# DhayaaAnbajagane/Baryonification

Hardware: AMD Instinct MI355X
Metric: halos/sec for BaryonifyShell NSIDE=1024 (1000000-halo synthetic catalog) (higher is better)
Workload: dtype f64 throughout in the parity-grade mode: f64 ring-row geometry, f64 pair math with 1e-11 elementary functions (fp32 seeds + one Newton step), f64 LDS accumulation, pix_offsets stored as two f32 arrays (hi + lo), f64 regrid geometry, f64 map

## Files before the change

### baryonification_amd/csrc/bfgx_regrid2.hpp

```cpp
#pragma once
#include "bfgx_kernels.hpp"
#include "bfgx_scatter2.hpp"

namespace bfgx {

template <typename real>
struct alignas(16) RegRowC {
    real z, sth, dphi, inv_dphi;
    real c0, s0;
    real inv_dth_up, inv_dth_dn;
};
template <>
struct alignas(16) RegRowC<double> { double inv_dth_up, inv_dth_dn; };
template <typename real> struct RowGeom { real z, sth, dphi, inv_dphi, c0, s0, inv_dth_up, inv_dth_dn; };
__device__ inline RowGeom<float> row_geom(const RegRow *, const RegRowC<float> *rowc, int t)
{
    const RegRowC<float> c = rowc[t];
    return RowGeom<float>{c.z, c.sth, c.dphi, c.inv_dphi, c.c0, c.s0, c.inv_dth_up, c.inv_dth_dn};
}
__device__ inline RowGeom<double> row_geom(const RegRow *rows, const RegRowC<double> *rowc, int t)
{
    const RegRow &r = rows[t];
    const RegRowC<double> c = rowc[t];
    return RowGeom<double>{r.z, r.sth, r.dphi, r.inv_dphi, r.c0, r.s0, c.inv_dth_up, c.inv_dth_dn};
}
__device__ inline float row_inv_dphi(const RegRow *, const RegRowC<float> *rowc, int t) { return rowc[t].inv_dphi; }
__device__ inline double row_inv_dphi(const RegRow *rows, const RegRowC<double> *, int t) { return rows[t].inv_dphi; }
__host__ __device__ inline size_t regrowc_bytes(size_t real_size) { return real_size == 4 ? sizeof(RegRowC<float>) : sizeof(RegRowC<double>); }

__device__ inline void regrid_targets_generic(const Hpx &h, const RegRow *rows, int LR, int rth0, int ti, int x,
                                                    double o0, double o1, double o2, int tr[4], int tk[4], double w[4])
{
    const int nl4 = (int)(4 * h.nside);
    const RegRow &rw = rows[ti];
    const double z = rw.z, sth = rw.sth;
    const double phi = ((double)(rw.ks + x) + (rw.shf ? 0.5 : 0.0)) * rw.dphi;
    double s, c;
    sincos_bounded(phi, s, c);
    const double nx = sth * c + o0, ny = sth * s + o1, nz = z + o2;
    const double xr = nx * c + ny * s, yr = ny * c - nx * s;
    const double inv = fast_rsq(nx * nx + ny * ny + nz * nz);
    const double zc = nz * inv;
    const double tq = yr * fast_rcp(xr);
    const double sn = fast_sqrt(xr * xr + yr * yr) * inv;
    const double q = sn * z - zc * sth;
    double theta, ph;
    if (xr > 0.0 && fabs(tq) <= 0.1 && fabs(q) <= 0.05) {
        ph = phi + atan_small(tq);
        theta = rw.theta + asin_small(q);
    } else {
        theta = atan2_generic(sn, zc);
        ph = atan2_generic(ny, nx);
    }
    if (ph < 0) ph += kTwoPi;
    if (ph >= kTwoPi) ph -= kTwoPi;
    int t1 = ti;
    while (t1 > 0 && theta < rows[t1].theta) --t1;
    while (t1 < LR + 1 && theta >= rows[t1 + 1].theta) ++t1;
    const bool in_window = (theta >= rows[t1].theta) && (t1 < LR + 1) && (theta < rows[t1 + 1].theta);
    const int ir1 = in_window ? rth0 + t1 : (int)ring_above(h, zc);
    const int ir2 = ir1 + 1;
    double theta1 = 0.0, theta2 = 0.0;
    for (int q4 = 0; q4 < 4; ++q4) { tr[q4] = 0; tk[q4] = 0; w[q4] = 0.0; }
#pragma unroll
    for (int half = 0; half < 2; ++half) {
        const int ir = half ? ir2 : ir1;
        if (half ? (ir < nl4) : (ir > 0)) {
            const int t2 = ir - rth0;
            int n2; double shd, invd, th;
            if (t2 >= 0 && t2 < LR + 2) {
                const RegRow &r2 = rows[t2];
                n2 = r2.nr; shd = r2.shf ? 0.5 : 0.0; invd = r2.inv_dphi; th = r2.theta;
            } else {
                n2 = ring_len(h, ir);
                const bool sh2 = (ir < h.nside) || (ir >= 3 * h.nside) || (((ir - (int)h.nside) & 1) == 0);
                shd = sh2 ? 0.5 : 0.0; invd = (double)n2 * kInvTwoPi; th = ring_theta_nolibm(h, ir);
            }
            const double tmp = ph * invd - shd;
            int j1 = (int)floor(tmp);
            const double w1 = tmp - (double)j1;
            int j2 = j1 + 1;
            if (j1 < 0) j1 += n2;
            if (j2 >= n2) j2 -= n2;
            tr[2 * half] = ir; tr[2 * half + 1] = ir;
            tk[2 * half] = j1; tk[2 * half + 1] = j2;
            w[2 * half] = 1.0 - w1; w[2 * half + 1] = w1;
            if (half) theta2 = th; else theta1 = th;
        }
    }
    if (ir1 == 0) {
        const double wtheta = theta / theta2;
        w[2] *= wtheta; w[3] *= wtheta;
        const double fac = (1.0 - wtheta) * 0.25;
        w[0] = fac; w[1] = fac; w[2] += fac; w[3] += fac;
        tr[0] = 1; tr[1] = 1; tk[0] = (tk[2] + 2) & 3; tk[1] = (tk[3] + 2) & 3;
    } else if (ir2 == nl4) {
        const double wtheta = (theta - theta1) / (kPi - theta1);
        w[0] *= (1.0 - wtheta); w[1] *= (1.0 - wtheta);
        const double fac = wtheta * 0.25;
        w[0] += fac; w[1] += fac; w[2] = fac; w[3] = fac;
        tr[2] = nl4 - 1; tr[3] = nl4 - 1; tk[2] = (tk[0] + 2) & 3; tk[3] = (tk[1] + 2) & 3;
    } else {
        const double wtheta = (theta - theta1) * fast_rcp(theta2 - theta1);
        w[0] *= (1.0 - wtheta); w[1] *= (1.0 - wtheta);
        w[2] *= wtheta; w[3] *= wtheta;
    }
}

__device__ inline float abs_(float v) { return __builtin_fabsf(v); }
__device__ inline double abs_(double v) { return __builtin_fabs(v); }
template <typename real> struct RMath;
template <> struct RMath<float> {
    static __device__ inline float rcp(float x) { const float y = __builtin_amdgcn_rcpf(x); return y * __builtin_fmaf(-x, y, 2.0f); }
    static __device__ inline float inv_norm(float e) { return fma_(e, fma_(e, fma_(e, fma_(e, 0.2734375f, -0.3125f), 0.375f), -0.5f), 1.0f); }
    static __device__ inline float sqrt1pm1(float t2) { return t2 * fma_(t2, fma_(t2, 0.0625f, -0.125f), 0.5f); }
    static __device__ inline float asin_(float q) { const float q2 = q * q; return q * fma_(q2, fma_(q2, fma_(q2, (float)(15.0 / 336.0), 0.075f), (float)(1.0 / 6.0)), 1.0f); }
    static __device__ inline float atan_(float t) { const float t2 = t * t; return t * fma_(t2, fma_(t2, fma_(t2, fma_(t2, (float)(1.0 / 9.0), (float)(-1.0 / 7.0)), 0.2f), (float)(-1.0 / 3.0)), 1.0f); }
};
template <> struct RMath<double> {
    static __device__ inline double rcp(double x) { return fast_rcp(x); }
    static __device__ inline double inv_norm(double e) { return fast_rsq(1.0 + e); }
    static __device__ inline double sqrt1pm1(double t2) { const double h = 1.0 + t2; return t2 * fast_rcp(1.0 + h * fast_rsq(h)); }
    static __device__ inline double asin_(double q) { return asin_small(q); }
    static __device__ inline double atan_(double t) { return atan_small(t); }
};

struct RMathE {
    static __device__ inline double rcp(double x) { const double y = (double)__builtin_amdgcn_rcpf((float)x); return __builtin_fma(y, __builtin_fma(-x, y, 1.0), y); }
    static __device__ inline double inv_norm(double e)
    {
        const double x = 1.0 + e, y = (double)__builtin_amdgcn_rsqf((float)x);
        const double h = 0.5 * y, r = __builtin_fma(-x * y, h, 0.5);
        return __builtin_fma(y, r, y);
    }
    static __device__ inline double sqrt1pm1(double t2) { return t2 * __builtin_fma(t2, __builtin_fma(t2, __builtin_fma(t2, __builtin_fma(t2, 7.0 / 256.0, -5.0 / 128.0), 0.0625), -0.125), 0.5); }
    static __device__ inline double asin_(double q) { const double q2 = q * q; return q * __builtin_fma(q2, __builtin_fma(q2, __builtin_fma(q2, 15.0 / 336.0, 0.075), 1.0 / 6.0), 1.0); }
    static __device__ inline double atan_(double t)
    {
        const double t2 = t * t;
        return t * __builtin_fma(t2, __builtin_fma(t2, __builtin_fma(t2, __builtin_fma(t2, __builtin_fma(t2, -1.0 / 11.0, 1.0 / 9.0), -1.0 / 7.0), 0.2), -1.0 / 3.0), 1.0);
    }
};

constexpr int kReachMax = 16;
constexpr int kReachColsMax = 256;

__host__ __device__ inline double regrid_cap(int64_t nside)
{
    const double c = 9.9 / (double)nside;
    return c < 0.02 ? c : 0.02;
}
__host__ __device__ inline int regrid_reach_rings(int64_t nside, double m)
{
    const double r = m * 1.5 * (double)nside;
    const int R = (r < (double)kReachMax ? (int)r : kReachMax) + 1;
    return R > kReachMax ? kReachMax : R;
}
__host__ __device__ inline double regrid_cap_for_rings(int64_t nside, int R)
{
    const double c = 0.999 * (double)R / (1.5 * (double)nside), cap = regrid_cap(nside);
    return (R >= kReachMax || c > cap) ? cap : c;
}

struct alignas(16) RowScan {
    int32_t start, nr, ks, span;
    float need2, cf2, lim2;
    int32_t klr;
};

struct FarList {
    unsigned long long *count;
    int64_t *pix;
    double *val;
    int64_t cap;
    int32_t *overflow;
};

struct ReachArgs {
    const int32_t *apron;
    double cap;
    double theta_first, theta_last;
};

constexpr int kWalkQ = 128;
constexpr int kWalkFar = (256 / kWave) * kWalkQ;
__host__ __device__ inline size_t regrid3_lds_bytes(int BR, int W, size_t real_size, bool walk = false, size_t acc_size = 0)
{
    if (acc_size == 0) acc_size = real_size;
    const size_t base = (size_t)BR * W * sizeof(double) + (size_t)(BR + 2 * kReachMax + 2) * (sizeof(RegRow) + regrowc_bytes(real_size)) + 16;
    if (!walk) return base;
    return base + (size_t)(BR + 2 * kReachMax + 2) * sizeof(RowScan) + (size_t)(256 / kWave) * kWalkQ * (sizeof(double) + sizeof(int32_t) + 3 * acc_size)
           + (size_t)(kWalkFar + 4) * sizeof(int32_t);
}

template <typename ACC>
__global__ void __launch_bounds__(256)
tile_reach_kernel(Hpx h, Tiling T, const ACC *__restrict__ offsets, float *__restrict__ tile_omax)
{
    __shared__ float red[256 / kWave];
    const int tile = blockIdx.x;
    const int band = T.tile_band[tile];
    const int nphi = T.band_nphi[band];
    const int tj = tile - T.band_tile0[band];
    const int nl4 = (int)(4 * h.nside);
    const int i0 = 1 + band * T.BR, i1 = min(i0 + T.BR, nl4);
    const int lane = threadIdx.x & (kWave - 1), wid = threadIdx.x / kWave;
    float m2 = 0.0f;
    for (int ring = i0 + wid; ring < i1; ring += 256 / kWave) {
        int64_t st, nr64; bool shf;
        ring_info_small(h, ring, st, nr64, shf);
        const int nr = (int)nr64, ks = tile_ks(tj, nr, nphi), ke = tile_ks(tj + 1, nr, nphi);
        const ACC *o = offsets + 3 * (st + ks);
        for (int x = lane; x < ke - ks; x += kWave) {
            const float a = (float)o[3 * x], b = (float)o[3 * x + 1], c = (float)o[3 * x + 2];
            m2 = fmaxf(m2, fma_(a, a, fma_(b, b, c * c)));
        }
    }
#pragma unroll
    for (int sft = kWave >> 1; sft > 0; sft >>= 1) m2 = fmaxf(m2, __shfl_down(m2, sft, kWave));
    if (lane == 0) red[wid] = m2;
    __syncthreads();
    if (threadIdx.x == 0) {
        for (int w = 1; w < 256 / kWave; ++w) m2 = fmaxf(m2, red[w]);
        tile_omax[tile] = m2;
    }
}

__global__ void __launch_bounds__(256)
tile_apron_kernel(Hpx h, Tiling T, const float *__restrict__ tile_omax, int rings, double cap, int tile0, int ntiles,
                  int32_t *__restrict__ apron, int32_t *__restrict__ todo, int32_t *__restrict__ lean = nullptr)
{
    const int i = blockIdx.x * 256 + threadIdx.x;
    bool is_lean = false;
    if (i < ntiles) {
    const int tile = tile0 + i;
    const int band = T.tile_band[tile];
    const int nphi = T.band_nphi[band];
    const int tj = tile - T.band_tile0[band];
    const int nl4 = (int)(4 * h.nside);
    float m = (float)cap;
    int R = rings;
    if (tile_omax != nullptr) {
        m = 0.0f;
        const int nb = (kReachMax + T.BR - 1) / T.BR;
        for (int db = -nb; db <= nb; ++db) {
            const int b2 = band + db;
            if (b2 < 0 || b2 >= T.nbands) continue;
            const int n2 = T.band_nphi[b2], t20 = T.band_tile0[b2];
            int lo = (int)(((int64_t)tj * n2) / nphi) - 1, hi = (int)(((int64_t)(tj + 1) * n2 + nphi - 1) / nphi) + 1;
            if (T.W < 32 || hi - lo >= n2) { lo = 0; hi = n2; }
            for (int t2 = lo; t2 < hi; ++t2) {
                const int u = t2 < 0 ? t2 + n2 : (t2 >= n2 ? t2 - n2 : t2);
                m = fmaxf(m, tile_omax[t20 + u]);
            }
        }
        const bool still = !(m > 0.0f);
        m = fminf(__builtin_sqrtf(m) * 1.001f, (float)cap);
        R = still ? 0 : regrid_reach_rings(h.nside, (double)m);
    }
    const int i0 = 1 + band * T.BR, i1 = min(i0 + T.BR, nl4);
    const int rlo = max(i0 - R, 1), rhi = min(i1 + R, nl4) - 1, ns = (int)h.nside;
    int nmin = 0x7fffffff, nmax = 0;
    float mc = 0.0f;
    const int probe[4] = {rlo, rhi, ns, 3 * ns};
#pragma unroll
    for (int q = 0; q < 4; ++q) {
        const int ring = probe[q];
        if (ring < rlo || ring > rhi) continue;
        double z, sth;
        ring_z_sth(h, ring, z, sth);
        const int nr = ring_len(h, ring);
        nmin = min(nmin, nr); nmax = max(nmax, nr);
        const float limf = fminf(m, (float)(0.09 * sth)), den = (float)sth - limf;
        if (den > 0.0f) mc = fmaxf(mc, limf / den * 1.02f * (float)nr * (float)kInvTwoPi);
    }
    const float kk = mc + (float)nmax / (float)nmin + 2.5f;
    apron[2 * tile] = R;
    apron[2 * tile + 1] = (nphi == 1) ? 0 : (kk < (float)kReachColsMax ? (int)kk + 1 : kReachColsMax);
    if (todo != nullptr && R > 1) todo[1 + atomicAdd(todo, 1)] = tile;
    is_lean = R <= 1;
    }
    if (lean != nullptr) {
        const unsigned long long m = __ballot(is_lean);
        if (m) {
            const int lane = threadIdx.x & (kWave - 1), leader = __ffsll((long long)m) - 1;
            int base = 0;
            if (lane == leader) base = atomicAdd(lean, __popcll(m));
            base = __shfl(base, leader, kWave);
            const int pos = base + __popcll(m & ((1ull << lane) - 1ull));
            if (is_lean && pos < ntiles) lean[1 + pos] = tile0 + i;
        }
    }
}

template <typename ACC>
__global__ void __launch_bounds__(256)
max_offset_kernel(int64_t n, const ACC *__restrict__ offsets, unsigned *__restrict__ out)
{
    float m2 = 0.0f;
    for (int64_t i = (int64_t)blockIdx.x * 256 + threadIdx.x; i < n; i += (int64_t)gridDim.x * 256) {
        const float a = (float)offsets[3 * i], b = (float)offsets[3 * i + 1], c = (float)offsets[3 * i + 2];
        m2 = fmaxf(m2, fma_(a, a, fma_(b, b, c * c)));
    }
#pragma unroll
    for (int sft = kWave >> 1; sft > 0; sft >>= 1) m2 = fmaxf(m2, __shfl_down(m2, sft, kWave));
    __shared__ float wm[256 / kWave];
    if ((threadIdx.x & (kWave - 1)) == 0) wm[threadIdx.x / kWave] = m2;
    __syncthreads();
    if (threadIdx.x == 0) {
        float m = 0.0f;
        for (int w = 0; w < 256 / kWave; ++w) m = fmaxf(m, wm[w]);
        if (m > 0.0f) atomicMax(out, __float_as_uint(m));
    }
}

__global__ void __launch_bounds__(1024)
max_bits_kernel(int n, const unsigned *__restrict__ v, unsigned *__restrict__ out)
{
    unsigned m = 0u;
    for (int i = threadIdx.x; i < n; i += 1024) m = max(m, v[i]);
#pragma unroll
    for (int sft = kWave >> 1; sft > 0; sft >>= 1) m = max(m, (unsigned)__shfl_down((int)m, sft, kWave));
    if ((threadIdx.x & (kWave - 1)) == 0 && m) atomicMax(out, m);
}

template <typename real, bool WALK, bool ECON = false>
__device__ inline bool regrid_gather_targets(const RegRow *rows, const RegRowC<real> *rowc, int NT, int ti, int x,
                                             real o0, real o1, real o2, int tt[4], int tk[4], real w[4])
{
    using RM = typename std::conditional<ECON, RMathE, RMath<real>>::type;
    using PMx = typename std::conditional<ECON, PMathE, PMath<real>>::type;
    const RowGeom<real> rc = row_geom(rows, rowc, ti);
    const RegRow &rw = rows[ti];
    real c, s;
    const real alpha = (real)x * rc.dphi;
    if (abs_(alpha) <= (real)0.45) {
        real sa, oma;
        PMx::sin_omc(alpha, sa, oma);
        c = rc.c0 - (rc.c0 * oma + rc.s0 * sa);
        s = rc.s0 - (rc.s0 * oma - rc.c0 * sa);
    } else {
        double s64, c64;
        sincos_bounded(((double)(rw.ks + x) + (rw.shf ? 0.5 : 0.0)) * rw.dphi, s64, c64);
        c = (real)c64; s = (real)s64;
    }
    const real a = o0 * c + o1 * s, b = o1 * c - o0 * s;
    const real xr = rc.sth + a;
    const real t = b * RM::rcp(xr);
    const real t2 = t * t;
    const real e = (real)2 * (rc.sth * a + rc.z * o2) + (a * a + b * b + o2 * o2);
    const real invn = RM::inv_norm(e);
    const real q = (fma_(a, rc.z, -(o2 * rc.sth)) + xr * rc.z * RM::sqrt1pm1(t2)) * invn;
    const real dth = RM::asin_(q);
    const real dph = RM::atan_(t);
    const bool down = dth >= (real)0;
    const real wq = down ? dth * rc.inv_dth_dn : -dth * rc.inv_dth_up;
    int t1 = ti;
    real wtheta;
    const bool near = wq < (real)1 && (down ? rc.inv_dth_dn : rc.inv_dth_up) > (real)0;
    if (!WALK || near) {
        wtheta = down ? wq : (real)1 - wq;
    } else {
        const double d = (double)dth, th0 = rw.theta;
        const int stp = (int)(wq < (real)(2 * kReachMax) ? wq : (real)(2 * kReachMax));
        t1 = down ? ti + stp : ti - 1 - stp;
        t1 = t1 < 0 ? 0 : (t1 > NT - 2 ? NT - 2 : t1);
        while (t1 + 2 < NT && d >= rows[t1 + 1].theta - th0) ++t1;
        while (t1 > 0 && d < rows[t1].theta - th0) --t1;
        const double lo = rows[t1].theta - th0, hi = rows[t1 + 1].theta - th0;
        if (!(d >= lo && d < hi) || rows[t1].nr == 0 || rows[t1 + 1].nr == 0) return false;
        wtheta = (real)((d - lo) * fast_rcp(hi - lo));
    }
    const int nro = rw.nr;
    int kown = rw.ks + x;
    if (kown < 0) kown += nro;
    if (kown >= nro) kown -= nro;
    auto other_ring = [&](int tr, int &j, real &wj) {
        const RegRow &rn = rows[tr];
        const double B = ((double)kown + (rw.shf ? 0.5 : 0.0)) * ((double)rn.nr * rw.dphi * kInvTwoPi) - (rn.shf ? 0.5 : 0.0);
        const double Bf = floor(B);
        const real wall = (real)(B - Bf) + dph * row_inv_dphi(rows, rowc, tr), f = __builtin_floor(wall);
        wj = wall - f; j = (int)Bf + (int)f;
    };
    const bool nr_ = !WALK || near;
    const bool x_upper = !nr_ || down;
    const int tx = nr_ ? ti : t1, ty = nr_ ? (down ? ti + 1 : ti - 1) : t1 + 1;
    int jx, jy; real wx, wy;
    if (nr_) {
        const real wall = dph * rc.inv_dphi, f = __builtin_floor(wall);
        wx = wall - f; jx = kown + (int)f;
    } else {
        other_ring(tx, jx, wx);
    }
    other_ring(ty, jy, wy);
    const int nrx = rows[tx].nr, nry = rows[ty].nr;
    int jx2 = jx + 1, jy2 = jy + 1;
    jx = jx < 0 ? jx + nrx : (jx >= nrx ? jx - nrx : jx);
    jx2 = jx2 < 0 ? jx2 + nrx : (jx2 >= nrx ? jx2 - nrx : jx2);
    jy = jy < 0 ? jy + nry : (jy >= nry ? jy - nry : jy);
    jy2 = jy2 < 0 ? jy2 + nry : (jy2 >= nry ? jy2 - nry : jy2);
    const real wtx = x_upper ? (real)1 - wtheta : wtheta, wty = (real)1 - wtx;
    tt[0] = tx; tt[1] = tx; tk[0] = jx; tk[1] = jx2;
    w[0] = ((real)1 - wx) * wtx; w[1] = wx * wtx;
    tt[2] = ty; tt[3] = ty; tk[2] = jy; tk[3] = jy2;
    w[2] = ((real)1 - wy) * wty; w[3] = wy * wty;
    return true;
}

__device__ inline double regrid_far_pixel(
    const Hpx &h, const RegRow *rows, int LR, int rth0, int ti, int x, double o0, double o1, double o2,
                                                double val, FarList far)
{
    int tr[4], tk[4];
    double w[4], tot = 0.0;
    regrid_targets_generic(h, rows, LR, rth0, ti, x, o0, o1, o2, tr, tk, w);
    const unsigned long long act = __ballot(1);
    const int rank = (int)__builtin_amdgcn_mbcnt_hi((unsigned)(act >> 32), __builtin_amdgcn_mbcnt_lo((unsigned)act, 0u));
    const int leader = __ffsll((long long)act) - 1;
    unsigned long long base = 0;
    if (rank == 0) base = atomicAdd(far.count, 4ull * (unsigned long long)__popcll(act));
    base = ((unsigned long long)(unsigned)__shfl((int)(base >> 32), leader, kWave) << 32) | (unsigned)__shfl((int)base, leader, kWave);
    for (int q4 = 0; q4 < 4; ++q4) {
        int64_t st_t, nr64; bool sh_t;
        ring_info_small(h, tr[q4], st_t, nr64, sh_t);
        const double v = w[q4] * val;
        const unsigned long long i = base + 4ull * (unsigned long long)rank + (unsigned long long)q4;
        if ((int64_t)i < far.cap) { far.pix[i] = st_t + tk[q4]; far.val[i] = v; } else atomicOr(far.overflow, 1);
        tot += v;
    }
    return tot;
}

constexpr int kK2Occ = 4;
template <typename ACC, typename real, int PASS, bool SPLIT = false>
__global__ void __launch_bounds__(256, kK2Occ)
tile_regrid3_kernel(Hpx h, Tiling T, const double *__restrict__ map_in, const ACC *__restrict__ offsets, const ACC *__restrict__ offsets_lo,
                    double *__restrict__ map_out, FarList far, ReachArgs reach, double *__restrict__ tile_sums, int tile_off, int ntiles,
                    int *__restrict__ todo, double *__restrict__ sums_out, int *__restrict__ lean_reset = nullptr)
{
    static_assert(!SPLIT || (sizeof(ACC) == 4 && sizeof(real) == 8), "split pix_offsets: fp32 halves, fp64 geometry");
    extern __shared__ __align__(16) unsigned char smem[];
    const int NTmax = T.BR + 2 * kReachMax + 2;
    double *acc = reinterpret_cast<double *>(smem);
    RegRow *rows = reinterpret_cast<RegRow *>(acc + T.BR * T.W);
    RegRowC<real> *rowc = reinterpret_cast<RegRowC<real> *>(rows + NTmax);
    const int tid = threadIdx.x;
    const int nl4 = (int)(4 * h.nside);
    if (PASS == 1 && lean_reset != nullptr && blockIdx.x == 0 && tid == 0) *lean_reset = 0;
    if (PASS == 1 && sums_out != nullptr && blockIdx.x == 0) {
        double sa = 0.0, sb = 0.0;
        for (int i = tid; i < ntiles; i += 256) { sa += tile_sums[2 * (int64_t)i]; sb += tile_sums[2 * (int64_t)i + 1]; }
#pragma unroll
        for (int sft = kWave >> 1; sft > 0; sft >>= 1) { sa += __shfl_down(sa, sft, kWave); sb += __shfl_down(sb, sft, kWave); }
        double *red = reinterpret_cast<double *>(smem);
        if ((tid & (kWave - 1)) == 0) { red[2 * (tid / kWave)] = sa; red[2 * (tid / kWave) + 1] = sb; }
        __syncthreads();
        if (tid == 0) {
            double ta = 0.0, tb = 0.0;
            for (int w = 0; w < 256 / kWave; ++w) { ta += red[2 * w]; tb += red[2 * w + 1]; }
            sums_out[0] = ta; sums_out[1] = tb;
        }
        __syncthreads();
    }
    if (PASS == 1 && *far.overflow == 0) {
        const unsigned long long n = *far.count;
        for (unsigned long long i = (unsigned long long)blockIdx.x * 256 + tid; i < n; i += (unsigned long long)gridDim.x * 256)
            atomicAdd(map_out + far.pix[i], far.val[i]);
        return;
    }
    const bool listed = (PASS == 2 || PASS == 0) && todo != nullptr;
    if (listed) ntiles = min(todo[0], ntiles);
    for (int blk = blockIdx.x; blk < ntiles; blk += ((PASS == 0 && !listed) ? ntiles : (int)gridDim.x)) {
    const int tile = listed ? todo[1 + blk] : ((tile_off < 0) ? T.tile_order[blk] : tile_off + blk);
    const int band = T.tile_band[tile];
    const int nphi = T.band_nphi[band];
    const int tj = tile - T.band_tile0[band];
    const int i0 = 1 + band * T.BR;
    const int i1 = min(i0 + T.BR, nl4);
    double sum_in = 0.0, sum_out = 0.0;
    __syncthreads();

    const int R = (PASS == 2) ? reach.apron[2 * tile] : 1;
    const int kap = (PASS == 1 || nphi == 1) ? 0 : reach.apron[2 * tile + 1];
    if (PASS == 0 && reach.apron[2 * tile] > 1) continue;
    if (PASS == 0 && reach.apron[2 * tile] == 0) {
        const int lane = tid & (kWave - 1), wid = tid / kWave;
        for (int rr = wid; rr < i1 - i0; rr += 256 / kWave) {
            int64_t st; int64_t nr64; bool shf_;
            ring_info_small(h, i0 + rr, st, nr64, shf_);
            const int ks = tile_ks(tj, (int)nr64, nphi), ke = tile_ks(tj + 1, (int)nr64, nphi);
            for (int k = ks + lane; k < ke; k += kWave) {
                const double v = map_in[st + k];
                const double dep = (v > 0.0) ? v : 0.0;
                map_out[st + k] = dep;
                sum_in += v; sum_out += dep;
            }
        }
        if (tile_sums) {
#pragma unroll
            for (int sft = kWave >> 1; sft > 0; sft >>= 1) { sum_in += __shfl_down(sum_in, sft, kWave); sum_out += __shfl_down(sum_out, sft, kWave); }
            if (lane == 0) { acc[2 * wid] = sum_in; acc[2 * wid + 1] = sum_out; }
            __syncthreads();
            if (tid == 0) {
                double sa_ = 0.0, sb_ = 0.0;
                for (int wv = 0; wv < 256 / kWave; ++wv) { sa_ += acc[2 * wv]; sb_ += acc[2 * wv + 1]; }
                tile_sums[2 * (int64_t)tile] = sa_; tile_sums[2 * (int64_t)tile + 1] = sb_;
            }
        }
        continue;
    }
    for (int i = tid; i < T.BR * T.W; i += 256) acc[i] = 0.0;
    const int NT = T.BR + 2 * R + 2;
    const int rth0 = i0 - R - 1;
    if (tid < NT) {
        const int ring = rth0 + tid;
        RegRow rw;
        rw.theta = (ring < 1) ? -1.0e300 : 1.0e300;
        rw.z = rw.sth = rw.dphi = rw.inv_dphi = rw.c0 = rw.s0 = 0.0;
        rw.start = 0; rw.nr = 0; rw.ks = 0; rw.ke = 0; rw.shf = 0; rw.lim2 = 0.0;
        if (ring >= 1 && ring <= nl4 - 1) {
            int64_t st, nr64; bool shf_;
            ring_info_small(h, ring, st, nr64, shf_);
            ring_z_sth(h, ring, rw.z, rw.sth);
            rw.theta = atan2_generic(rw.sth, rw.z);
            rw.start = st; rw.nr = (int)nr64; rw.shf = shf_ ? 1 : 0;
            rw.dphi = kTwoPi / (double)rw.nr;
            rw.inv_dphi = (double)rw.nr * kInvTwoPi;
            rw.ks = tile_ks(tj, rw.nr, nphi);
            rw.ke = tile_ks(tj + 1, rw.nr, nphi);
            sincos_bounded(((double)rw.ks + (shf_ ? 0.5 : 0.0)) * rw.dphi, rw.s0, rw.c0);
            const double lim = fmin(fmin(reach.cap, 0.09 * rw.sth), 0.999 * fmin(rw.theta - reach.theta_first, reach.theta_last - rw.theta));
            rw.lim2 = (lim > 0.0 && ring > 1 && ring < nl4 - 1) ? (double)(float)(lim * lim) : 0.0;
        }
        rows[tid] = rw;
    }
    __syncthreads();
    if (tid < NT) {
        const RegRow &rw = rows[tid];
        RegRowC<real> rc;
        if constexpr (sizeof(real) == 4) {
            rc.z = (real)rw.z; rc.sth = (real)rw.sth; rc.dphi = (real)rw.dphi; rc.inv_dphi = (real)rw.inv_dphi;
            rc.c0 = (real)rw.c0; rc.s0 = (real)rw.s0;
        }
        rc.inv_dth_up = (real)0; rc.inv_dth_dn = (real)0;
        if (rw.nr > 0) {
            if (tid > 0 && rows[tid - 1].nr > 0) rc.inv_dth_up = (real)(1.0 / (rw.theta - rows[tid - 1].theta));
            if (tid < NT - 1 && rows[tid + 1].nr > 0) rc.inv_dth_dn = (real)(1.0 / (rows[tid + 1].theta - rw.theta));
        }
        rowc[tid] = rc;
        if (PASS == 2) {
            RowScan *scan = reinterpret_cast<RowScan *>(rowc + NTmax);
            const int T0 = R + 1, T1 = R + (i1 - i0);
            double need = 0.0;
            if (tid < T0 - 1 && rows[T0 - 1].nr > 0) need = rows[T0 - 1].theta - rw.theta;
            else if (tid > T1 + 1 && rows[T1 + 1].nr > 0) need = rw.theta - rows[T1 + 1].theta;
            const float nf = (rw.nr > 0 && need > 0.0) ? (float)(0.999 * need) : 0.0f;
            const double den = rw.sth - fast_sqrt(rw.lim2);
            const float cf = (rw.nr > 0 && den > 0.0) ? (float)(1.02 * rw.inv_dphi / den) : 3.0e18f;
            const int span = rw.ke - rw.ks, rest = rw.nr - span;
            const int kl = min(kap, rest >> 1), kr = min(kap, rest - kl);
            RowScan rs;
            rs.start = (int32_t)rw.start; rs.nr = rw.nr; rs.ks = rw.ks; rs.span = span;
            rs.need2 = nf * nf; rs.cf2 = cf * cf; rs.lim2 = (float)rw.lim2;
            rs.klr = kl | (kr << 10) | ((tid >= T0 && tid <= T1) ? (1 << 20) : 0);
            scan[tid] = rs;
        }
    }
    if (PASS == 2 && tid == 0) reinterpret_cast<int32_t *>(reinterpret_cast<RowScan *>(rowc + NTmax) + NTmax)[0] = 0;
    __syncthreads();
    auto far_add = [&](int64_t p, double v) {
        if (PASS != 1) {
            const unsigned long long i = atomicAdd(far.count, 1ull);
            if ((int64_t)i < far.cap) { far.pix[i] = p; far.val[i] = v; } else atomicOr(far.overflow, 1);
            sum_out += v;
        } else {
            atomicAdd(map_out + p, v);
        }
    };

    const int NR = T.BR + 2 * R;
    int maxspan = 0, nrmin = 0x7fffffff, nrmax = 1;
    for (int i = 1; i <= NR; ++i) {
        maxspan = max(maxspan, rows[i].ke - rows[i].ks);
        if (PASS == 2 && rows[i].nr > 0) { nrmin = min(nrmin, rows[i].nr); nrmax = max(nrmax, rows[i].nr); }
    }
    const int LWs = maxspan + 2 * kap;
    const unsigned inv_lws = (unsigned)((0x100000000ull + (unsigned)LWs - 1u) / (unsigned)LWs);
    using OT = typename std::conditional<SPLIT, double, ACC>::type;
    struct Src { int ti, x; bool ok, own; double val; OT o0, o1, o2; float hsq; };
    auto fetch = [&](int idx) {
        Src sx;
        sx.ok = false; sx.own = false; sx.ti = 0; sx.x = 0; sx.val = 0.0; sx.o0 = sx.o1 = sx.o2 = (OT)0; sx.hsq = 0.0f;
        if (idx < NR * LWs) {
            const int r = (int)__umulhi((unsigned)idx, inv_lws), x = idx - r * LWs - kap;
            const RegRow &rw = rows[r + 1];
            const int span = rw.ke - rw.ks, rest = rw.nr - span;
            const int kl = min(kap, rest >> 1), kr = min(kap, rest - kl);
            if (rw.nr > 0 && x >= -kl && x < span + kr) {
                int k = rw.ks + x;
                if (k < 0) k += rw.nr;
                if (k >= rw.nr) k -= rw.nr;
                const int64_t p = rw.start + k;
                sx.own = (r >= R) && (r < R + (i1 - i0)) && (x >= 0) && (x < span);
                if (PASS != 1 || sx.own) {
                    sx.ok = true; sx.ti = r + 1; sx.x = x;
                    sx.val = map_in[p];
                    if (SPLIT) {
                        const ACC h0 = offsets[3 * p + 0], h1 = offsets[3 * p + 1], h2 = offsets[3 * p + 2];
                        const ACC l0 = offsets_lo[3 * p + 0], l1 = offsets_lo[3 * p + 1], l2 = offsets_lo[3 * p + 2];
                        sx.o0 = (OT)((double)h0 + (double)l0); sx.o1 = (OT)((double)h1 + (double)l1); sx.o2 = (OT)((double)h2 + (double)l2);
                        sx.hsq = (float)fma_(h0, h0, fma_(h1, h1, h2 * h2));
                    } else {
                    sx.o0 = offsets[3 * p + 0]; sx.o1 = offsets[3 * p + 1]; sx.o2 = offsets[3 * p + 2];
                    }
                }
            }
        }
        return sx;
    };
    if constexpr (PASS == 2) {
        const int lane = tid & (kWave - 1), wid = __builtin_amdgcn_readfirstlane(tid / kWave);
        const RowScan *scan = reinterpret_cast<const RowScan *>(rowc + NTmax);
        int32_t *nfar = reinterpret_cast<int32_t *>(const_cast<RowScan *>(scan) + NTmax), *farq = nfar + 4;
        double *qval = reinterpret_cast<double *>(farq + kWalkFar) + wid * kWalkQ;
        using QT = typename std::conditional<SPLIT, ACC, real>::type;
        QT *qo = reinterpret_cast<QT *>(reinterpret_cast<double *>(farq + kWalkFar) + (256 / kWave) * kWalkQ) + wid * 3 * kWalkQ;
        int32_t *qpos = reinterpret_cast<int32_t *>(reinterpret_cast<QT *>(reinterpret_cast<double *>(farq + kWalkFar) + (256 / kWave) * kWalkQ)
                                                    + (256 / kWave) * 3 * kWalkQ) + wid * kWalkQ;
        const float colslack = 2.5f + (float)nrmax / (float)nrmin;
        const int nown = i1 - i0, total = NR * LWs;
        auto deposit = [&](int ti, int x, QT q0, QT q1, QT q2, double val) {
            int tt[4], tk[4];
            real w[4];
            real o0 = (real)q0, o1 = (real)q1, o2 = (real)q2;
            if (SPLIT) {
                const RegRow &rs_ = rows[ti];
                int k = rs_.ks + x;
                k += (k < 0) ? rs_.nr : 0;
                k -= (k >= rs_.nr) ? rs_.nr : 0;
                const int64_t p = rs_.start + k;
                o0 += (real)offsets_lo[3 * p + 0]; o1 += (real)offsets_lo[3 * p + 1]; o2 += (real)offsets_lo[3 * p + 2];
            }
            if (!regrid_gather_targets<real, true, SPLIT>(rows, rowc, NT, ti, x, o0, o1, o2, tt, tk, w)) return;
#pragma unroll
            for (int q4 = 0; q4 < 4; ++q4) {
                const int rr = tt[q4] - (R + 1);
                if (rr >= 0 && rr < nown) {
                    const RegRow &rt = rows[tt[q4]];
                    if (tk[q4] >= rt.ks && tk[q4] < rt.ke) {
                        const double v = (double)w[q4] * val;
                        atomicAdd(acc + rr * T.W + (tk[q4] - rt.ks), v);
                    }
                }
            }
        };
        auto far_from = [&](int pk) {
            const int ti = pk >> 16, x = (pk & 0xffff) - kap;
            const RegRow &rw = rows[ti];
            int k = rw.ks + x;
            if (k < 0) k += rw.nr;
            if (k >= rw.nr) k -= rw.nr;
            const int64_t p = rw.start + k;
            double f0 = (double)offsets[3 * p + 0], f1 = (double)offsets[3 * p + 1], f2 = (double)offsets[3 * p + 2];
            if (SPLIT) { f0 += (double)offsets_lo[3 * p + 0]; f1 += (double)offsets_lo[3 * p + 1]; f2 += (double)offsets_lo[3 * p + 2]; }
            sum_out += regrid_far_pixel(h, rows, NT - 2, rth0, ti, x, f0, f1, f2, map_in[p], far);
        };
        int32_t *fq = farq + wid * kWalkQ;
        int fn = 0;
        int qn = 0;
        constexpr int U = 2;
        const int64_t pdummy = rows[R + 1].start + rows[R + 1].ks;
        for (int base = wid * kWave; base < total; base += 256 * U) {
            int cpos[U], cx[U], cspan[U];
            bool cin[U], cown[U];
            float cneed2[U], ccf2[U], clim2[U];
            ACC ca0[U], ca1[U], ca2[U];
            double cval[U];
#pragma unroll
            for (int u = 0; u < U; ++u) {
                const int idx = base + u * 256 + lane, idc = min(idx, total - 1);
                const int r = (int)__umulhi((unsigned)idc, inv_lws), x = idc - r * LWs - kap;
                const RowScan rs = scan[r + 1];
                cx[u] = x; cpos[u] = ((r + 1) << 16) | (x + kap); cspan[u] = rs.span;
                cneed2[u] = rs.need2; ccf2[u] = rs.cf2; clim2[u] = rs.lim2;
                cin[u] = idx < total && rs.nr > 0 && x >= -(rs.klr & 1023) && x < rs.span + ((rs.klr >> 10) & 1023);
                cown[u] = cin[u] && (rs.klr >> 20) && x >= 0 && x < rs.span;
                int k = rs.ks + x;
                k += (k < 0) ? rs.nr : 0;
                k -= (k >= rs.nr) ? rs.nr : 0;
                const int64_t p = cin[u] ? (int64_t)(rs.start + k) : pdummy;
                ca0[u] = offsets[3 * p + 0]; ca1[u] = offsets[3 * p + 1]; ca2[u] = offsets[3 * p + 2];
                cval[u] = map_in[p];
            }
            bool cpush[U], cfar[U];
#pragma unroll
            for (int u = 0; u < U; ++u) {
                const int x = cx[u];
                if (cown[u]) sum_in += cval[u];
                const QT o0 = (QT)ca0[u], o1 = (QT)ca1[u], o2 = (QT)ca2[u];
                const QT osq = fma_(o0, o0, fma_(o1, o1, o2 * o2));
                const bool live = cin[u] && cval[u] > 0.0;
                const bool gathered = osq < (QT)clim2[u];
                const int dc = x < 0 ? -x : (x >= cspan[u] ? x - cspan[u] + 1 : 0);
                const float g = (float)dc - colslack, of = (float)osq;
                const bool reaches = cown[u] || (of >= cneed2[u] && (g <= 0.0f || of * ccf2[u] >= g * g));
                cpush[u] = live && gathered && reaches;
                cfar[u] = live && !gathered && cown[u];
            }
#pragma unroll
            for (int u = 0; u < U; ++u) {
                const unsigned long long m = __ballot(cpush[u]);
                if (m == 0ull) continue;
                if (cpush[u]) {
                    const int sl = qn + (int)__builtin_amdgcn_mbcnt_hi((unsigned)(m >> 32), __builtin_amdgcn_mbcnt_lo((unsigned)m, 0u));
                    qval[sl] = cval[u]; qo[sl] = (QT)ca0[u]; qo[kWalkQ + sl] = (QT)ca1[u]; qo[2 * kWalkQ + sl] = (QT)ca2[u]; qpos[sl] = cpos[u];
                }
                qn += __popcll(m);
                __builtin_amdgcn_wave_barrier();
                if (qn >= kWave) {
                    qn -= kWave;
                    const int sl = qn + lane, pk = qpos[sl];
                    deposit(pk >> 16, (pk & 0xffff) - kap, qo[sl], qo[kWalkQ + sl], qo[2 * kWalkQ + sl], qval[sl]);
                    __builtin_amdgcn_wave_barrier();
                }
            }
#pragma unroll
            for (int u = 0; u < U; ++u) {
                const unsigned long long m = __ballot(cfar[u]);
                if (m == 0ull) continue;
                if (cfar[u]) fq[fn + (int)__builtin_amdgcn_mbcnt_hi((unsigned)(m >> 32), __builtin_amdgcn_mbcnt_lo((unsigned)m, 0u))] = cpos[u];
                fn += __popcll(m);
                __builtin_amdgcn_wave_barrier();
                if (fn >= kWave) {
                    fn -= kWave;
                    far_from(fq[fn + lane]);
                    __builtin_amdgcn_wave_barrier();
                }
            }
        }
        if (lane < qn) {
            const int pk = qpos[lane];
            deposit(pk >> 16, (pk & 0xffff) - kap, qo[lane], qo[kWalkQ + lane], qo[2 * kWalkQ + lane], qval[lane]);
        }
        if (lane < fn) far_from(fq[lane]);
    } else {
    auto handle = [&](const Src &cur) {
        if (cur.ok && cur.own) sum_in += cur.val;
        if (!cur.ok || !(cur.val > 0.0)) return;
        const double val = cur.val;
        const real o0 = (real)cur.o0, o1 = (real)cur.o1, o2 = (real)cur.o2;
        const real osq = fma_(o0, o0, fma_(o1, o1, o2 * o2));
        const bool gathered = SPLIT ? (cur.hsq < (float)rows[cur.ti].lim2) : ((double)osq < rows[cur.ti].lim2);
        if (gathered) {
            if (PASS == 1) return;
            int tt[4], tk[4];
            real w[4];
            if (!regrid_gather_targets<real, false, SPLIT>(rows, rowc, NT, cur.ti, cur.x, o0, o1, o2, tt, tk, w)) return;
#pragma unroll
            for (int q4 = 0; q4 < 4; ++q4) {
                const int rr = tt[q4] - (R + 1);
                if (rr >= 0 && rr < i1 - i0) {
                    const RegRow &rt = rows[tt[q4]];
                    if (tk[q4] >= rt.ks && tk[q4] < rt.ke) {
                        const double v = (double)w[q4] * val;
                        atomicAdd(acc + rr * T.W + (tk[q4] - rt.ks), v);
                    }
                }
            }
        } else if (cur.own) {
            int tr[4], tk[4];
            double w[4];
            regrid_targets_generic(h, rows, NT - 2, rth0, cur.ti, cur.x, (double)cur.o0, (double)cur.o1, (double)cur.o2, tr, tk, w);
            for (int q4 = 0; q4 < 4; ++q4) {
                int64_t st_t, nr64; bool sh_t;
                ring_info_small(h, tr[q4], st_t, nr64, sh_t);
                far_add(st_t + tk[q4], w[q4] * val);
            }
        }
    };
    for (int idx = tid; idx < NR * LWs; idx += 512) {
        const Src a = fetch(idx), b = fetch(idx + 256);
        handle(a);
        handle(b);
    }
    }
    if (PASS == 1) continue;
    __syncthreads();

    const int lane = tid & (kWave - 1), wid = tid / kWave;
    for (int rr = wid; rr < i1 - i0; rr += 256 / kWave) {
        const RegRow &rt = rows[rr + R + 1];
        double *dst = map_out + rt.start + rt.ks;
        const int n = rt.ke - rt.ks;
        for (int xx = lane; xx < n; xx += kWave) {
            const double v = acc[rr * T.W + xx];
            dst[xx] = v;
            sum_out += v;
        }
    }
    if (tile_sums) {
        __syncthreads();
#pragma unroll
        for (int sft = kWave >> 1; sft > 0; sft >>= 1) { sum_in += __shfl_down(sum_in, sft, kWave); sum_out += __shfl_down(sum_out, sft, kWave); }
        if (lane == 0) { acc[2 * wid] = sum_in; acc[2 * wid + 1] = sum_out; }
        __syncthreads();
        if (tid == 0) {
            double sa_ = 0.0, sb_ = 0.0;
            for (int wv = 0; wv < 256 / kWave; ++wv) { sa_ += acc[2 * wv]; sb_ += acc[2 * wv + 1]; }
            tile_sums[2 * (int64_t)tile] = sa_; tile_sums[2 * (int64_t)tile + 1] = sb_;
        }
    }
    __syncthreads();
    }
}

__global__ void __launch_bounds__(256)
regrid_far_local_kernel(FarList far, double *__restrict__ out_slice, int64_t p0, int64_t p1, unsigned long long *__restrict__ foreign,
                        int ntiles = 0, const double *__restrict__ tile_sums = nullptr, double *__restrict__ sums = nullptr)
{
    if (tile_sums != nullptr && blockIdx.x == gridDim.x - 1) {
        __shared__ double sa[256 / kWave], sb[256 / kWave];
        double xa = 0.0, xb = 0.0;
        for (int t = threadIdx.x; t < ntiles; t += 256) { xa += tile_sums[2 * t]; xb += tile_sums[2 * t + 1]; }
#pragma unroll
        for (int sft = kWave >> 1; sft > 0; sft >>= 1) { xa += __shfl_down(xa, sft, kWave); xb += __shfl_down(xb, sft, kWave); }
        const int lane = threadIdx.x & (kWave - 1), wid = threadIdx.x / kWave;
        if (lane == 0) { sa[wid] = xa; sb[wid] = xb; }
        __syncthreads();
        if (threadIdx.x == 0) {
            double ta = 0.0, tb = 0.0;
            for (int w = 0; w < 256 / kWave; ++w) { ta += sa[w]; tb += sb[w]; }
            sums[0] = ta; sums[1] = tb;
        }
    }
    unsigned long long n = *far.count;
    if ((int64_t)n > far.cap) n = (unsigned long long)far.cap;
    for (unsigned long long i = (unsigned long long)blockIdx.x * blockDim.x + threadIdx.x; i < n; i += (unsigned long long)gridDim.x * blockDim.x) {
        const int64_t p = far.pix[i];
        if (p >= p0 && p < p1) atomicAdd(out_slice + (p - p0), far.val[i]);
        else if (foreign) atomicAdd(foreign, 1ull);
    }
}

}
```

Baseline: 907.9 million.

## Add fp32 pretest filter and compact position-only queues to f64 regrid walk

For the f64 non-split walk path, pushed candidate pixels are split into direct (owned or single-tile) and candidate queues storing only positions. Candidates run a cheap fp32 geometric pretest against per-row precomputed bounds (theta window and phi range) before the full f64 deposit, and survivors are compacted into the deposit queue. Offsets and values are reloaded from global memory at deposit time instead of being stored in LDS, which shrinks queue LDS usage. This trades extra global reloads and fp32 math for skipping expensive f64 target computation on pixels that cannot land in the tile, with a risk of wrongly dropping pixels near the fp32 tolerance margins.

```diff
diff --git a/baryonification_amd/csrc/bfgx_regrid2.hpp b/baryonification_amd/csrc/bfgx_regrid2.hpp
--- a/baryonification_amd/csrc/bfgx_regrid2.hpp
+++ b/baryonification_amd/csrc/bfgx_regrid2.hpp
@@ -184,12 +184,21 @@
 
 constexpr int kWalkQ = 128;
 constexpr int kWalkFar = (256 / kWave) * kWalkQ;
+template <typename real, bool SPLIT> constexpr bool kWalkPre = sizeof(real) == 8 && !SPLIT;
+constexpr int kWalkQP = 192;
+struct PreRow {
+    float z, sth, c0, s0;
+    float rel0;
+    float dlo, dhi;
+};
 __host__ __device__ inline size_t regrid3_lds_bytes(int BR, int W, size_t real_size, bool walk = false, size_t acc_size = 0)
 {
     if (acc_size == 0) acc_size = real_size;
     const size_t base = (size_t)BR * W * sizeof(double) + (size_t)(BR + 2 * kReachMax + 2) * (sizeof(RegRow) + regrowc_bytes(real_size)) + 16;
     if (!walk) return base;
-    return base + (size_t)(BR + 2 * kReachMax + 2) * sizeof(RowScan) + (size_t)(256 / kWave) * kWalkQ * (sizeof(double) + sizeof(int32_t) + 3 * acc_size)
+    const bool pre = real_size == 8 && acc_size == 8;
+    const size_t queues = pre ? (size_t)kWalkQP * 2 * sizeof(int32_t) : (size_t)kWalkQ * (sizeof(double) + sizeof(int32_t) + 3 * acc_size);
+    return base + (size_t)(BR + 2 * kReachMax + 2) * (sizeof(RowScan) + (pre ? sizeof(PreRow) : 0)) + (size_t)(256 / kWave) * queues
            + (size_t)(kWalkFar + 4) * sizeof(int32_t);
 }
 
@@ -564,6 +573,21 @@
             rs.need2 = nf * nf; rs.cf2 = cf * cf; rs.lim2 = (float)rw.lim2;
             rs.klr = kl | (kr << 10) | ((tid >= T0 && tid <= T1) ? (1 << 20) : 0);
             scan[tid] = rs;
+            if constexpr (kWalkPre<real, SPLIT>) {
+                int32_t *nfar_ = reinterpret_cast<int32_t *>(scan + NTmax);
+                PreRow *pre = reinterpret_cast<PreRow *>(nfar_ + 4 + kWalkFar + (256 / kWave) * 2 * kWalkQP);
+                int nrmin_ = 0x7fffffff;
+                for (int i = 1; i <= T.BR + 2 * R; ++i) if (rows[i].nr > 0) nrmin_ = min(nrmin_, rows[i].nr);
+                const double colm = (1.5 + 1.0 / 16.0) * kTwoPi / (double)nrmin_, thm = 1.0 / (24.0 * (double)h.nside);
+                const double w2 = kTwoPi / (double)nphi + 2.0 * colm;
+                const double num = ((double)rw.ks + (rw.shf ? 0.5 : 0.0)) * (double)nphi - (double)tj * (double)rw.nr;
+                PreRow pr;
+                pr.z = (float)rw.z; pr.sth = (float)rw.sth; pr.c0 = (float)rw.c0; pr.s0 = (float)rw.s0;
+                pr.rel0 = (nphi == 1 || w2 > 5.0 || rw.nr == 0) ? 1.0f : (float)(num * rw.dphi / (double)nphi + colm);
+                pr.dlo = (float)(rows[T0 - 1].theta - rw.theta - thm); pr.dhi = (float)(rows[T1 + 1].theta - rw.theta + thm);
+                pre[tid] = pr;
+                if (tid == 0) reinterpret_cast<float *>(nfar_)[1] = (float)w2;
+            }
         }
     }
     if (PASS == 2 && tid == 0) reinterpret_cast<int32_t *>(reinterpret_cast<RowScan *>(rowc + NTmax) + NTmax)[0] = 0;
@@ -622,24 +646,28 @@
         const int lane = tid & (kWave - 1), wid = __builtin_amdgcn_readfirstlane(tid / kWave);
         const RowScan *scan = reinterpret_cast<const RowScan *>(rowc + NTmax);
         int32_t *nfar = reinterpret_cast<int32_t *>(const_cast<RowScan *>(scan) + NTmax), *farq = nfar + 4;
-        double *qval = reinterpret_cast<double *>(farq + kWalkFar) + wid * kWalkQ;
+        constexpr bool PRE = kWalkPre<real, SPLIT>;
         using QT = typename std::conditional<SPLIT, ACC, real>::type;
-        QT *qo = reinterpret_cast<QT *>(reinterpret_cast<double *>(farq + kWalkFar) + (256 / kWave) * kWalkQ) + wid * 3 * kWalkQ;
-        int32_t *qpos = reinterpret_cast<int32_t *>(reinterpret_cast<QT *>(reinterpret_cast<double *>(farq + kWalkFar) + (256 / kWave) * kWalkQ)
-                                                    + (256 / kWave) * 3 * kWalkQ) + wid * kWalkQ;
+        int32_t *qbase = farq + kWalkFar;
+        int32_t *rpos = qbase + wid * kWalkQP;
+        double *qval = PRE ? nullptr : reinterpret_cast<double *>(qbase) + wid * kWalkQ;
+        QT *qo = PRE ? nullptr : reinterpret_cast<QT *>(reinterpret_cast<double *>(qbase) + (256 / kWave) * kWalkQ) + wid * 3 * kWalkQ;
+        int32_t *qpos = PRE ? qbase + (256 / kWave) * kWalkQP + wid * kWalkQP
+                            : reinterpret_cast<int32_t *>(reinterpret_cast<QT *>(reinterpret_cast<double *>(qbase) + (256 / kWave) * kWalkQ) + (256 / kWave) * 3 * kWalkQ) + wid * kWalkQ;
         const float colslack = 2.5f + (float)nrmax / (float)nrmin;
         const int nown = i1 - i0, total = NR * LWs;
         auto deposit = [&](int ti, int x, QT q0, QT q1, QT q2, double val) {
             int tt[4], tk[4];
             real w[4];
             real o0 = (real)q0, o1 = (real)q1, o2 = (real)q2;
-            if (SPLIT) {
+            if (SPLIT || PRE) {
                 const RegRow &rs_ = rows[ti];
                 int k = rs_.ks + x;
                 k += (k < 0) ? rs_.nr : 0;
                 k -= (k >= rs_.nr) ? rs_.nr : 0;
                 const int64_t p = rs_.start + k;
-                o0 += (real)offsets_lo[3 * p + 0]; o1 += (real)offsets_lo[3 * p + 1]; o2 += (real)offsets_lo[3 * p + 2];
+                if (PRE) { o0 = (real)offsets[3 * p + 0]; o1 = (real)offsets[3 * p + 1]; o2 = (real)offsets[3 * p + 2]; val = map_in[p]; }
+                if (SPLIT) { o0 += (real)offsets_lo[3 * p + 0]; o1 += (real)offsets_lo[3 * p + 1]; o2 += (real)offsets_lo[3 * p + 2]; }
             }
             if (!regrid_gather_targets<real, true, SPLIT>(rows, rowc, NT, ti, x, o0, o1, o2, tt, tk, w)) return;
 #pragma unroll
@@ -665,12 +693,43 @@
             if (SPLIT) { f0 += (double)offsets_lo[3 * p + 0]; f1 += (double)offsets_lo[3 * p + 1]; f2 += (double)offsets_lo[3 * p + 2]; }
             sum_out += regrid_far_pixel(h, rows, NT - 2, rth0, ti, x, f0, f1, f2, map_in[p], far);
         };
+        const PreRow *pre = reinterpret_cast<const PreRow *>(qbase + (256 / kWave) * 2 * kWalkQP);
+        auto pretest = [&](int pk) -> bool {
+            const int ti = pk >> 16, x = (pk & 0xffff) - kap;
+            const RegRow &rw = rows[ti];
+            const PreRow pr = pre[ti];
+            int k = rw.ks + x;
+            k += (k < 0) ? rw.nr : 0;
+            k -= (k >= rw.nr) ? rw.nr : 0;
+            const int64_t p = rw.start + k;
+            const float o0 = (float)offsets[3 * p + 0], o1 = (float)offsets[3 * p + 1], o2 = (float)offsets[3 * p + 2];
+            const float alpha = (float)x * (float)rw.dphi;
+            bool drop = false;
+            if (abs_(alpha) <= 0.45f) {
+                float sa, oma;
+                PMath<float>::sin_omc(alpha, sa, oma);
+                const float c = pr.c0 - (pr.c0 * oma + pr.s0 * sa), s_ = pr.s0 - (pr.s0 * oma - pr.c0 * sa);
+                const float a = o0 * c + o1 * s_, b = o1 * c - o0 * s_;
+                const float xr = pr.sth + a;
+                const float t = b * RMath<float>::rcp(xr);
+                if (xr > 0.0f && abs_(t) <= 0.1f) {
+                    const float e = 2.0f * (pr.sth * a + pr.z * o2) + (a * a + b * b + o2 * o2);
+                    const float q = (fma_(a, pr.z, -(o2 * pr.sth)) + xr * pr.z * RMath<float>::sqrt1pm1(t * t)) * RMath<float>::inv_norm(e);
+                    const float dth = RMath<float>::asin_(q), rel = pr.rel0 + alpha + RMath<float>::atan_(t);
+                    drop = dth < pr.dlo || dth > pr.dhi || rel < 0.0f || rel > reinterpret_cast<const float *>(nfar)[1];
+                }
+            }
+            return !drop;
+        };
+        int rn = 0;
         int32_t *fq = farq + wid * kWalkQ;
         int fn = 0;
         int qn = 0;
         constexpr int U = 2;
         const int64_t pdummy = rows[R + 1].start + rows[R + 1].ks;
-        for (int base = wid * kWave; base < total; base += 256 * U) {
+        for (int base = wid * kWave; PRE || base < total; base += 256 * U) {
+            const bool last = PRE && base >= total;
+            if (!last) {
             int cpos[U], cx[U], cspan[U];
             bool cin[U], cown[U];
             float cneed2[U], ccf2[U], clim2[U];
@@ -711,6 +770,13 @@
             for (int u = 0; u < U; ++u) {
                 const unsigned long long m = __ballot(cpush[u]);
                 if (m == 0ull) continue;
+                if constexpr (PRE) {
+                    const bool direct = cpush[u] && (cown[u] || nphi == 1);
+                    const unsigned long long md = __ballot(direct), mc = m & ~md;
+                    if (direct) qpos[qn + (int)__builtin_amdgcn_mbcnt_hi((unsigned)(md >> 32), __builtin_amdgcn_mbcnt_lo((unsigned)md, 0u))] = cpos[u];
+                    else if (cpush[u]) rpos[rn + (int)__builtin_amdgcn_mbcnt_hi((unsigned)(mc >> 32), __builtin_amdgcn_mbcnt_lo((unsigned)mc, 0u))] = cpos[u];
+                    qn += __popcll(md); rn += __popcll(mc);
+                } else {
                 if (cpush[u]) {
                     const int sl = qn + (int)__builtin_amdgcn_mbcnt_hi((unsigned)(m >> 32), __builtin_amdgcn_mbcnt_lo((unsigned)m, 0u));
                     qval[sl] = cval[u]; qo[sl] = (QT)ca0[u]; qo[kWalkQ + sl] = (QT)ca1[u]; qo[2 * kWalkQ + sl] = (QT)ca2[u]; qpos[sl] = cpos[u];
@@ -723,6 +789,7 @@
                     deposit(pk >> 16, (pk & 0xffff) - kap, qo[sl], qo[kWalkQ + sl], qo[2 * kWalkQ + sl], qval[sl]);
                     __builtin_amdgcn_wave_barrier();
                 }
+                }
             }
 #pragma unroll
             for (int u = 0; u < U; ++u) {
@@ -737,10 +804,38 @@
                     __builtin_amdgcn_wave_barrier();
                 }
             }
-        }
+            }
+            if constexpr (PRE) {
+                __builtin_amdgcn_wave_barrier();
+                const int full = last ? 1 : kWave;
+#pragma nounroll
+                while (qn >= full || rn >= full) {
+                    if (qn >= kWave || rn < full) {
+                        const int n = min(qn, kWave);
+                        qn -= n;
+                        if (lane < n) {
+                            const int pk = qpos[qn + lane];
+                            deposit(pk >> 16, (pk & 0xffff) - kap, (QT)0, (QT)0, (QT)0, 0.0);
+                        }
+                    } else {
+                        const int n = min(rn, kWave);
+                        rn -= n;
+                        const int pk = lane < n ? rpos[rn + lane] : 0;
+                        const bool keep = lane < n && pretest(pk);
+                        const unsigned long long mk = __ballot(keep);
+                        if (keep) qpos[qn + (int)__builtin_amdgcn_mbcnt_hi((unsigned)(mk >> 32), __builtin_amdgcn_mbcnt_lo((unsigned)mk, 0u))] = pk;
+                        qn += __popcll(mk);
+                    }
+                    __builtin_amdgcn_wave_barrier();
+                }
+                if (last) break;
+            }
+        }
+        if constexpr (!PRE) {
         if (lane < qn) {
             const int pk = qpos[lane];
             deposit(pk >> 16, (pk & 0xffff) - kap, qo[lane], qo[kWalkQ + lane], qo[2 * kWalkQ + lane], qval[lane]);
+        }
         }
         if (lane < fn) far_from(fq[lane]);
     } else {
```

After: 904.3 million. No clear change (-0.4%).
